# bkpcoding/distributed_ML_pytorch

Measured on AMD Instinct MI355X. Metric: samples/sec (whole node) ResNet-18 ASGD at 1/2/4/8 MI355X; time-to-target-loss, higher is better.
Workload: dtype bf16; 1 GPU; model=resnet18 (CIFAR stem), global_batch=512, per_gpu_batch=512, image=3x32x32, parallelism=asgd-local-ps x1, n_push=10, n_pull=10, staleness=1, push_combine=sum, hip_graph=True, master_dtype=fp32, wire_dtype=fp32

## Files before the change

### distributed_ml_pytorch_amd/csrc/bind/conv.cpp

```cpp
#include "util.h"

namespace dmp::bind {
namespace {

struct ConvGeom {
  int B, CI, H, W, CO, R, S, OH, OW;
};

ConvGeom geom_of(const Tensor& x, const Tensor& w, int64_t OH, int64_t OW) {
  return {(int)x.size(0), (int)x.size(1), (int)x.size(2), (int)x.size(3), (int)w.size(0),
          (int)w.size(2), (int)w.size(3), (int)OH, (int)OW};
}

bool halo_takes(int64_t cfg, int H, int W, int C, int R, int S, int64_t stride, int64_t pad) {
  return cfg >= dmp::conv_halo_base() && cfg < dmp::conv_halo_base() + dmp::conv_num_halo_configs() &&
         stride == 1 && pad == 1 &&
         dmp::conv_halo_ok((int)cfg, H, W, C, R, S, (int)stride, (int)pad);
}

ConvGeom conv_geom(const Tensor& x, const Tensor& w, int64_t stride, int64_t pad,
                   int64_t halo_cfg = -1) {
  TORCH_CHECK(x.dim() == 4 && w.dim() == 4, "conv: 4-D tensors expected");
  TORCH_CHECK(w.size(1) == x.size(1), "conv: weight/input channel mismatch");
  TORCH_CHECK(stride >= 1 && pad >= 0, "conv: bad stride/pad");
// ... 360 lines not shown
  return config_table(dmp::conv_num_configs(), dmp::conv_config_info, 5);
}

std::vector<int64_t> conv_halo_configs(int64_t H, int64_t W, int64_t C, int64_t R, int64_t S,
                                       int64_t stride, int64_t pad) {
  std::vector<int64_t> out;
  config_ids(out, dmp::conv_halo_base(), dmp::conv_num_halo_configs(), [&](int c) {
    return dmp::conv_halo_ok(c, (int)H, (int)W, (int)C, (int)R, (int)S, (int)stride, (int)pad);
  });
  return out;
}

std::vector<int64_t> conv_dgrad_s2_configs(int64_t H, int64_t W, int64_t OH, int64_t OW,
                                           int64_t CO, int64_t CI, int64_t R, int64_t S,
                                           int64_t stride, int64_t pad) {
  std::vector<int64_t> out;
  config_ids(out, dmp::conv_dgrad_s2_base(), dmp::conv_dgrad_s2_num_configs(), [&](int c) {
    return dmp::conv_dgrad_s2_ok(c, (int)H, (int)W, (int)OH, (int)OW, (int)CO, (int)CI, (int)R,
                                 (int)S, (int)stride, (int)pad);
  });
  return out;
}

std::vector<int64_t> conv_wgrad_halo_configs(int64_t B, int64_t H, int64_t W, int64_t CI,
                                             int64_t CO, int64_t R, int64_t S, int64_t stride,
                                             int64_t pad) {
  std::vector<int64_t> out;
  for (int base : {dmp::conv_wgrad_halo_base(), dmp::conv_wgrad_halo_slab_base()})
    config_ids(out, base, dmp::conv_wgrad_num_halo_configs(), [&](int c) {
      return dmp::conv_wgrad_halo_ok(c, (int)B, (int)H, (int)W, (int)CI, (int)CO, (int)R, (int)S,
                                     (int)stride, (int)pad);
    });
  return out;
}

}

void bind_conv(pybind11::module_& m) {
  m.def("conv_fwd", &conv_fwd, "NHWC bf16 implicit-GEMM conv forward (+BN partials)",
        py::arg("x"), py::arg("w"), py::arg("stride"), py::arg("pad"), py::arg("want_stats"),
        py::arg("cfg") = -1, py::arg("slots") = py::none(), py::arg("bias") = py::none(),
        py::arg("relu") = false, py::arg("addend") = py::none());
  m.def("conv_dgrad", &conv_dgrad, "NHWC bf16 implicit-GEMM conv data gradient", py::arg("dy"),
        py::arg("w"), py::arg("H"), py::arg("W"), py::arg("stride"), py::arg("pad"),
        py::arg("cfg") = -1, py::arg("wt") = py::none(), py::arg("addend") = py::none(),
        py::arg("addend_sub") = false, py::arg("addend_mask") = py::none());
  m.def("subsample2", &subsample2, "x[:, :, ::2, ::2] of a channels_last bf16 activation",
        py::arg("x"));
  m.def("add_subsampled2", &add_subsampled2, "dx[:, :, ::2, ::2] += xs in place",
        py::arg("dx"), py::arg("xs"));
  m.def("conv_weight_transpose_batched", &conv_weight_transpose_batched,
        "transpose every conv weight of a flat bf16 shadow in one launch");
  m.def("conv_wgrad", &conv_wgrad, "NHWC bf16 conv weight gradient (fp32 accumulate)",
        py::arg("dy"), py::arg("x"), py::arg("dw"), py::arg("stride"), py::arg("pad"),
        py::arg("cfg") = -1, py::arg("dbias") = py::none());
  m.def("conv_configs", &conv_configs, "[(id, BM, BN, BK, threads)] of the compiled conv tiles");
  m.def("conv_wgrad_halo_configs", &conv_wgrad_halo_configs,
        "3x3 stride-1 / stride-2 halo wgrad cfg ids applicable to (B, H, W, CI, CO, R, S, stride, pad)");
  m.def("conv_dgrad_s2_configs", &conv_dgrad_s2_configs,
        "3x3/stride-2 halo data-gradient cfg ids for (H, W, OH, OW, CO, CI, R, S, stride, pad)");
  m.def("conv_halo_configs", &conv_halo_configs,
        "3x3/stride-1 halo-tile cfg ids applicable to (H, W, C, R, S, stride, pad)");
  m.def("conv_halo_pm", [](bool on) { return dmp::conv_halo_pm(on); },
        "position-major halo tiles on 4 x 4 maps: set the process-wide switch, return the "
        "previous value (never inside a graph capture)", py::arg("on"));
  m.def("conv_halo_pm_ok",
        [](int64_t cfg, int64_t H, int64_t W, int64_t C, int64_t R, int64_t S, int64_t stride,
           int64_t pad) {
          return dmp::conv_halo_pm_ok((int)cfg, (int)H, (int)W, (int)C, (int)R, (int)S, (int)stride,
                                      (int)pad);
        },
        "halo cfg id runs position-major on (H, W, C, R, S, stride, pad) when the switch is on");
  m.def("stem_supported", [](int64_t H, int64_t W) { return dmp::stem_supported((int)H, (int)W); },
        "ImageNet 7x7/2 stem kernel applies to an H x W input");
  m.def("stem_fwd", &stem_fwd, "ImageNet stem conv forward (+BN partials) via space-to-depth",
        py::arg("x"), py::arg("w"), py::arg("want_stats"), py::arg("slots") = py::none(),
        py::arg("bias") = py::none(), py::arg("relu") = false);
  m.def("stem_wgrad", &stem_wgrad, "ImageNet stem conv weight gradient (fp32 +=)", py::arg("dy"),
        py::arg("xs"), py::arg("dw"));
  m.def("conv_small_fwd", &conv_small_fwd, "few-input-channel conv forward (+BN partials)",
        py::arg("x"), py::arg("w"), py::arg("stride"), py::arg("pad"), py::arg("want_stats"),
        py::arg("slots") = py::none());
  m.def("conv_small_wgrad", &conv_small_wgrad, "few-input-channel conv weight gradient (fp32 +=)",
        py::arg("dy"), py::arg("x"), py::arg("dw"), py::arg("stride"), py::arg("pad"));
  m.def("stem3_route", &stem3_route,
        "conv_small_fwd / conv_small_wgrad run the MFMA stem kernels for this geometry",
        py::arg("CI"), py::arg("R"), py::arg("S"), py::arg("CO"), py::arg("stride"),
        py::arg("pad"), py::arg("W"));
  m.def("stem3_bn_bwd_scratch_floats", [] { return (int64_t)dmp::stem3_bn_bwd_scratch_floats(); },
        "fp32 elements of stem3_bn_bwd's persistent scratch");
  m.def("stem3_bn_bwd", &stem3_bn_bwd,
        "CIFAR stem: BN + ReLU backward and conv weight gradient in one pass (all +=)",
        py::arg("dy"), py::arg("x0"), py::arg("x"), py::arg("stats"), py::arg("gamma"),
        py::arg("dgamma"), py::arg("dbeta"), py::arg("dw"), py::arg("scratch"),
        py::arg("zero_buf") = py::none(), py::arg("blocks") = 0);
  m.def("im2col", &im2col, "NHWC patch rows [B*OH*OW, Kp], k = (r, s, ci), zero-padded",
        py::arg("x"), py::arg("R"), py::arg("S"), py::arg("stride"), py::arg("pad"), py::arg("Kp"));
  m.def("col2im", &col2im, "gather-form inverse of im2col -> channels_last dX", py::arg("dcols"),
        py::arg("B"), py::arg("CI"), py::arg("H"), py::arg("W"), py::arg("R"), py::arg("S"),
        py::arg("stride"), py::arg("pad"));
}

}
```

### distributed_ml_pytorch_amd/csrc/conv_wgrad.hip

```cpp
#include "common.h"
#include "halo_plan.h"
#include "mfma_prims.h"

#ifndef DMP_ABLATE
#define DMP_ABLATE 0
#endif

namespace dmp {


struct WgradArgs {
  const u16* dy;
  const u16* x;
  float* dw;
  int B, GH, GW, CI, OH, OW, CO, R, S, stride, pad;
  long long P;
  int p_chunk;
  float* dbias;
  float* slab;
  int xcd;
};

template <int ROWE>
__device__ __forceinline__ int wg_f(int row) {
  if constexpr (ROWE == 128) return (row & 3) | (((row >> 3) & 1) << 2);
  else return ((row >> 1) & 1) | (((row >> 3) & 1) << 1);
}
template <int ROWE>
__device__ __forceinline__ int wg_off(int row, int col) {
  return row * ROWE + ((((col >> 4) ^ wg_f<ROWE>(row))) << 4) + (col & 15);
}

// ... 398 lines not shown
    float* park = reinterpret_cast<float*>(lds_w);
    if (grp == 1) {
#pragma unroll
      for (int t = 0; t < NT; ++t)
#pragma unroll
        for (int i = 0; i < 4; ++i)
          *reinterpret_cast<f32x4*>(park + ((wc * NT * 4 + t * 4 + i) * 64 + lane) * 4) = acc[t][i];
    }
    __syncthreads();
    if (grp == 1) return;
#pragma unroll
    for (int t = 0; t < NT; ++t)
#pragma unroll
      for (int i = 0; i < 4; ++i)
        acc[t][i] += *reinterpret_cast<const f32x4*>(park + ((wc * NT * 4 + t * 4 + i) * 64 + lane) * 4);
  }
  const long long K = 9LL * C;
  const int ci = ci0 + wc * 16 + (lane & 15);
#pragma unroll
  for (int t = 0; t < NT; ++t)
#pragma unroll
    for (int i = 0; i < 4; ++i)
#pragma unroll
      for (int rr = 0; rr < 4; ++rr) {
        const int co = co0 + i * 16 + 4 * (lane >> 4) + rr;
        float* dst = a.dw + (long long)co * K + ((r0 + t / 3) * 3 + t % 3) * C + ci;
        if (atomic == 1) atomicAdd(dst, acc[t][i][rr]);
        else if (atomic == 0) *dst += acc[t][i][rr];
        else if (atomic == 3) a.slab[(long long)bz * CO * K + (dst - a.dw)] = acc[t][i][rr];
        else *dst = acc[t][i][rr];
      }
}

bool conv_wgrad_halo_ok(int cfg, int B, int H, int W, int CI, int CO, int R, int S, int stride,
                        int pad) {
  const WgradHaloPlan p = plan_wgrad_halo(cfg, B, H, W, CI, CO, R, S, stride, pad);
  return p.ok && (cfg < kWhSlabBase || p.slab_elems > 0);
}
long long conv_wgrad_halo_slab_elems(int cfg, int B, int H, int W, int CI, int CO, int R, int S,
                                     int stride, int pad) {
  return plan_wgrad_halo(cfg, B, H, W, CI, CO, R, S, stride, pad).slab_elems;
}
int conv_wgrad_halo_base() { return kWhBase; }
int conv_wgrad_halo_slab_base() { return kWhSlabBase; }
int conv_wgrad_num_halo_configs() { return kNumWhConfigs; }

__global__ void __launch_bounds__(256) wgrad_slab_reduce_kernel(const float* __restrict__ slab,
                                                                float* __restrict__ dw,
                                                                long long n4, int splits) {
  __shared__ float4 red[16][16];
  const int lx = threadIdx.x & 15, ly = threadIdx.x >> 4;
  const long long v = (long long)blockIdx.x * 16 + lx;
  const float4* s4 = reinterpret_cast<const float4*>(slab);
  float4 t = {0.f, 0.f, 0.f, 0.f};
  if (v < n4) {
    int sp = ly;
#pragma unroll 4
    for (; sp < splits; sp += 16) {
      const float4 u = s4[sp * n4 + v];
      t.x += u.x; t.y += u.y; t.z += u.z; t.w += u.w;
    }
  }
  red[ly][lx] = t;
  __syncthreads();
  if (ly == 0 && v < n4) {
#pragma unroll
// ... 11 lines not shown
static void launch_wgrad_halo_t(const WgradArgs& a, const WgradHaloGeom& g, size_t lds, int splits,
                                hipStream_t s) {
  static int diag = -1;
  allow_max_dynamic_lds<conv_wgrad_halo_kernel<BM, NS, TR, PG, S2>>();
  if (diag < 0) {
    const char* e = getenv("DMP_WGRAD_HALO_DIAG");
    diag = (e && e[0] == 's') ? 1 : 0;
  }
  const dim3 grid((unsigned)(a.CI / 64), (unsigned)(a.CO / 64 * (3 / TR)), (unsigned)splits);
  const int mode = diag ? 2 : (splits > 1 ? (a.slab != nullptr ? 3 : 1) : 0);
  hipLaunchKernelGGL((conv_wgrad_halo_kernel<BM, NS, TR, PG, S2>), grid, dim3(256 * PG), lds, s, a,
                     g, mode);
  if (mode == 3) {
    const long long n4 = (long long)a.CO * 9 * a.CI / 4;
    hipLaunchKernelGGL(wgrad_slab_reduce_kernel, dim3((unsigned)((n4 + 15) / 16)), dim3(256), 0,
                       s, a.slab, a.dw, n4, splits);
  }
}

template <int NS, int TR>
static void launch_wgrad_halo_bm(int bm, const WgradArgs& a, const WgradHaloGeom& g, size_t lds,
                                 int sp, hipStream_t s) {
  if constexpr (TR == 1) {
    if (bm == 224) {
      launch_wgrad_halo_t<224, NS, 1>(a, g, lds, sp, s);
      return;
    }
  }
  if (bm == 64) launch_wgrad_halo_t<64, NS, TR>(a, g, lds, sp, s);
  else if (TR == 3 || bm == 128) launch_wgrad_halo_t<128, NS, TR>(a, g, lds, sp, s);
  else launch_wgrad_halo_t<(TR == 3 ? 128 : 256), NS, TR>(a, g, lds, sp, s);
}

template <int BNW, int WM, int WN, int BMW = 64>
static void launch_wgrad_variant(const WgradArgs& a, dim3 grid, int bp, int ns, hipStream_t s) {
  if (bp == 32) {
    if (ns == 3) hipLaunchKernelGGL((conv_wgrad_kernel<BNW, WM, WN, 32, 3, BMW>), grid, dim3(256), 0, s, a);
    else hipLaunchKernelGGL((conv_wgrad_kernel<BNW, WM, WN, 32, 2, BMW>), grid, dim3(256), 0, s, a);
  } else {
    if (ns == 3) hipLaunchKernelGGL((conv_wgrad_kernel<BNW, WM, WN, 64, 3, BMW>), grid, dim3(256), 0, s, a);
    else hipLaunchKernelGGL((conv_wgrad_kernel<BNW, WM, WN, 64, 2, BMW>), grid, dim3(256), 0, s, a);
  }
}

void launch_conv_wgrad(const u16* dy, const u16* x, float* dw, int B, int H, int W, int CI,
                       int OH, int OW, int CO, int R, int S, int stride, int pad, int cfg,
                       hipStream_t s, float* dbias, float* slab) {
  WgradArgs a{dy, x, dw, B, H, W, CI, OH, OW, CO, R, S, stride, pad, (long long)B * OH * OW, 0,
              dbias, nullptr};
  if (cfg >= kWhSlabBase) {
    if (slab != nullptr) a.slab = slab;
    else cfg -= kWhSlabBase - kWhBase;
  }
  if (cfg >= kWhBase && dbias == nullptr) {
    if (const WgradHaloPlan p = plan_wgrad_halo(cfg, B, H, W, CI, CO, R, S, stride, pad); p.ok) {
      const WgradHaloGeom& g = p.g;
      const int bm = p.bm, ns = p.ns, tr = p.tr, pg = p.pg, sp = p.splits;
      const size_t lds = p.lds;
      if (stride == 2) {
        if (pg == 2) {
          if (bm == 128) launch_wgrad_halo_t<128, 2, 1, 2, true>(a, g, lds, sp, s);
          else launch_wgrad_halo_t<256, 2, 1, 2, true>(a, g, lds, sp, s);
        } else if (ns == 2) {
          if (bm == 64) launch_wgrad_halo_t<64, 2, 1, 1, true>(a, g, lds, sp, s);
          else if (bm == 128) launch_wgrad_halo_t<128, 2, 1, 1, true>(a, g, lds, sp, s);
          else launch_wgrad_halo_t<256, 2, 1, 1, true>(a, g, lds, sp, s);
        } else {
          if (bm == 64) launch_wgrad_halo_t<64, 3, 1, 1, true>(a, g, lds, sp, s);
          else if (bm == 128) launch_wgrad_halo_t<128, 3, 1, 1, true>(a, g, lds, sp, s);
          else launch_wgrad_halo_t<256, 3, 1, 1, true>(a, g, lds, sp, s);
        }
        return;
      }
      if (pg == 2) {
        if (bm == 128) launch_wgrad_halo_t<128, 2, 1, 2>(a, g, lds, sp, s);
        else launch_wgrad_halo_t<256, 2, 1, 2>(a, g, lds, sp, s);
      } else if (tr == 3) {
        if (ns == 2) launch_wgrad_halo_bm<2, 3>(bm, a, g, lds, sp, s);
        else launch_wgrad_halo_bm<3, 3>(bm, a, g, lds, sp, s);
      } else {
        if (ns == 2) launch_wgrad_halo_bm<2, 1>(bm, a, g, lds, sp, s);
        else if (ns == 3) launch_wgrad_halo_bm<3, 1>(bm, a, g, lds, sp, s);
        else launch_wgrad_halo_bm<4, 1>(bm, a, g, lds, sp, s);
      }
      return;
// ... 36 lines not shown
```

### distributed_ml_pytorch_amd/csrc/halo_plan.h

```cpp
#pragma once

#include <cstddef>

#include "halo_pm.h"

namespace dmp {

constexpr int kMaxDynamicLds = 160 * 1024;

struct HaloGeom {
  int TH, TB, HROWS, A_INS, MV;
  int W2, PI, PSW;
};

struct HaloPGeom {
  int TH, TB, HROWS, APW, AINS, ntiles;
  int xform;
  float xs, xh, xlo;
  int stagger;
};

struct WgradHaloGeom {
  int TH, TB, THX, XROWS, XPW, ntiles, tiles_per_split, MV;
};

constexpr int kHaloAPW = 8;
constexpr int kHpAPW = 12;
constexpr int hp_apw_max(int nw) { return nw == 8 ? 8 : kHpAPW; }
constexpr int kWhXPW = 12;

struct HaloTiling {
  bool ok;
  int TH, TB, MV;
};

inline HaloTiling halo_tiling(int bm, int H, int W, bool padded) {
  HaloTiling t{};
// ... 239 lines not shown
  if (stride != 1 && !(s2 && tr == 1 && H % 2 == 0 && W % 2 == 0 && ns <= 3 && kWhBM[var] == 0))
    return p;
  if (tr == 3 && bm > 128) return p;
  const int XW = W;
  if (s2) { H /= 2; W /= 2; }
  const HaloTiling t = halo_tiling(bm, H, W, true);
  if (!t.ok) return p;
  WgradHaloGeom& h = p.g;
  h.TH = t.TH;
  h.TB = t.TB;
  h.MV = t.MV;
  h.THX = h.TH + tr - 1;
  h.XROWS = h.TB * h.THX * (XW + 2);
  h.XPW = ((h.XROWS + 7) / 8 + 4 * pg - 1) / (4 * pg);
  if (h.XPW > kWhXPW || h.THX + 1 > 127 || h.TB > 0x7fff) return p;
  if ((ns - 2) * (bm / 32 + h.XPW) > 40) return p;
  const long long M = (long long)B * H * W;
  if (2LL * M * (CO > CI ? CO : CI) * (s2 ? 4 : 1) >= (1LL << 31)) return p;
  h.ntiles = (int)((M + h.MV - 1) / h.MV);
  const int per = (CI / 64) * (CO / 64) * (3 / tr);
  int sp = target / per;
  if (sp < 1) sp = 1;
  if (sp > h.ntiles) sp = h.ntiles;
  h.tiles_per_split = (h.ntiles + sp - 1) / sp;
  p.splits = (h.ntiles + h.tiles_per_split - 1) / h.tiles_per_split;
  const size_t stage = (size_t)bm * 64 + (size_t)h.XPW * 4 * pg * 512;
  p.lds = (size_t)ns * stage * 2;
  p.ok = p.lds <= (size_t)kMaxDynamicLds;
  if (p.ok && slab && p.splits > 1 && wh_slab_variant(var))
    p.slab_elems = (long long)p.splits * CO * R * S * CI;
  return p;
}

}
```

### distributed_ml_pytorch_amd/csrc/launchers.h

```cpp
#pragma once
#include <hip/hip_runtime_api.h>

#include "bn_slots.h"
#include <stdint.h>

namespace dmp {

void launch_asgd_fused_step(const float* g, float* p, float* acc, float* mom, uint16_t* w16,
                            long long n, float lr, float wd, float momentum, float dampening,
                            bool nesterov, hipStream_t s);
int optim_hyper_words();
void launch_optim_hyper(float* hyper, const float* g, float* partial, long long n, hipStream_t s);
void launch_asgd_fused_step_dev(const float* g, float* p, float* acc, float* mom, uint16_t* w16,
                                long long n, const float* hyper, float wd, float momentum,
                                float dampening, bool nesterov, hipStream_t s);
void launch_adamw_fused_step(const float* g, float* p, float* acc, float* m, float* v,
                             uint16_t* w16, const uint8_t* decay, long long n, const float* hyper,
                             float wd, float eps, hipStream_t s);
struct Wire {
  enum Kind { kF32, kBF16, kMX8 } kind;
  const void* data;
};
void launch_ps_apply(float* shard, Wire delta, uint16_t* mirror, long long n, float scale,
                     bool atomic, hipStream_t s, const float* factor = nullptr);
// ... 136 lines not shown
void launch_dropout_mask(uint8_t* mask, long long nmask, float p, unsigned long long seed,
                         const long long* offset, hipStream_t s);
void launch_dropout_apply_bf16(const uint16_t* x, const uint8_t* mask, uint16_t* y, long long n,
                               float scale, int mode, long long inner, int C, hipStream_t s);
void launch_dropout_apply_f32(const float* x, const uint8_t* mask, float* y, long long n,
                              float scale, int mode, long long inner, int C, hipStream_t s);

void launch_drop_path_draw(float* table, long long* state, const long long* thr,
                           const float* scale, int branches, int B, unsigned long long seed,
                           hipStream_t s);
void launch_drop_path_rows(const uint16_t* x, const float* rscale, uint16_t* y, long long per,
                           long long nvec, hipStream_t s);

int conv_num_configs();
void conv_config_info(int cfg, int* info);
int conv_default_config(long long M, int CO);
int conv_fwd_num_mblocks(long long M, int CO, int cfg);
int conv_num_halo_configs();
bool conv_dgrad_s2_ok(int cfg, int H, int W, int OH, int OW, int K, int N, int R, int S, int stride,
                      int pad);
int conv_dgrad_s2_base();
int conv_dgrad_s2_num_configs();
int conv_halo_base();
bool conv_halo_ok(int cfg, int H, int W, int C, int R, int S, int stride, int pad);
bool conv_halo_pm(bool on);
bool conv_halo_pm_ok(int cfg, int H, int W, int C, int R, int S, int stride, int pad);
int conv_wgrad_halo_base();
int conv_wgrad_num_halo_configs();
bool conv_wgrad_halo_ok(int cfg, int B, int H, int W, int CI, int CO, int R, int S, int stride,
                        int pad);
int conv_wgrad_halo_slab_base();
long long conv_wgrad_halo_slab_elems(int cfg, int B, int H, int W, int CI, int CO, int R, int S,
                                     int stride, int pad);
void launch_conv_fwd(const uint16_t* x, const uint16_t* w, uint16_t* y, float* part, int B, int H,
                     int W, int CI, int OH, int OW, int CO, int R, int S, int stride, int pad,
                     int cfg, hipStream_t s, const float* bias = nullptr, bool relu = false,
                     const uint16_t* addend = nullptr);
void launch_conv_dgrad(const uint16_t* dy, const uint16_t* wt, uint16_t* dx, int B, int H, int W,
                       int CI, int OH, int OW, int CO, int R, int S, int stride, int pad, int cfg,
                       hipStream_t s, const uint16_t* addend = nullptr, bool addend_sub = false,
                       const uint8_t* addend_mask = nullptr);
void launch_subsample2(const uint16_t* x, uint16_t* xs, int B, int H, int W, int C,
                       hipStream_t s);
void launch_add_subsampled2(uint16_t* dx, const uint16_t* xs, int B, int H, int W, int C,
                            hipStream_t s);
void launch_conv_weight_transpose(const uint16_t* w, uint16_t* wt, int CO, int RS, int CI,
                                  hipStream_t s);
void launch_conv_wgrad(const uint16_t* dy, const uint16_t* x, float* dw, int B, int H, int W,
                       int CI, int OH, int OW, int CO, int R, int S, int stride, int pad, int cfg,
                       hipStream_t s, float* dbias = nullptr, float* slab = nullptr);

bool stem3_supported(int CI, int R, int S, int CO, int stride, int pad, int W);
void launch_stem3_fwd(const uint16_t* x, int xbytes, int sb, int sh, int sw, int sc,
                      const uint16_t* w, uint16_t* y, float* part, int B, int H, int W, int CI,
                      hipStream_t s);
void launch_stem3_wgrad(const uint16_t* dy, const uint16_t* x, int xbytes, int sb, int sh, int sw,
                        int sc, float* dw, int B, int H, int W, int CI, hipStream_t s);
int stem3_bn_bwd_scratch_floats();
int stem3_bn_bwd_steps(long long P, int target);
long long stem3_bn_bwd_blocks(long long P, int target);
void launch_stem3_bn_bwd(const uint16_t* dy, const uint16_t* x0, const uint16_t* x, int xbytes,
                         int sb, int sh, int sw, int sc, const float* stats, const float* gamma,
                         float* dgamma, float* dbeta, float* dw, float* scratch, float* zero_buf,
                         int B, int H, int W, int CI, int blocks, hipStream_t s);
int conv_small_max_k();
long long conv_small_fwd_blocks(long long P);
// ... 61 lines not shown
```

Before: 146,700 samples/s.

## Add position-major halo weight-gradient kernel for 4x4 and 8x8 maps

Adds a new 3x3 stride-1 wgrad kernel for 4x4 and 8x8 feature maps. It stages tiles position-major, grouping 32 images per column, and skips MFMAs for dead padding taps, so only (3W-2)^2 of the 9W^2 products are computed. Work is split across row offsets with its own split planner and slab reduction. Reads go through transposed LDS reads with an XOR swizzle meant to avoid bank conflicts. It is on by default through an env switch and routes eligible halo configs away from the existing halo kernel, at the cost of more code paths and a new planner that could pick poorer splits.

```diff
diff --git a/distributed_ml_pytorch_amd/csrc/bind/conv.cpp b/distributed_ml_pytorch_amd/csrc/bind/conv.cpp
--- a/distributed_ml_pytorch_amd/csrc/bind/conv.cpp
+++ b/distributed_ml_pytorch_amd/csrc/bind/conv.cpp
@@ -416,6 +416,15 @@
                                      (int)stride, (int)pad);
     });
   return out;
+}
+
+bool conv_wgrad_pm_ok(int64_t cfg, int64_t B, int64_t H, int64_t W, int64_t CI, int64_t CO,
+                      int64_t R, int64_t S, int64_t stride, int64_t pad) {
+  if (std::max({cfg, B, H, W, CI, CO, R, S, stride, pad}) >= (int64_t(1) << 30) ||
+      std::min({cfg, B, H, W, CI, CO, R, S, stride, pad}) < 0)
+    return false;
+  return dmp::conv_wgrad_pm_ok((int)cfg, (int)B, (int)H, (int)W, (int)CI, (int)CO, (int)R, (int)S,
+                               (int)stride, (int)pad);
 }
 
 }
@@ -455,6 +464,13 @@
                                       (int)pad);
         },
         "halo cfg id runs position-major on (H, W, C, R, S, stride, pad) when the switch is on");
+  m.def("conv_wgrad_pm", [](bool on) { return dmp::conv_wgrad_pm(on); },
+        "position-major halo weight gradient on 4 x 4 / 8 x 8 maps: set the process-wide "
+        "switch, return the previous value (never inside a graph capture)", py::arg("on"));
+  m.def("conv_wgrad_pm_ok", &conv_wgrad_pm_ok,
+        "halo wgrad cfg id runs position-major on (B, H, W, CI, CO, R, S, stride, pad) when the "
+        "switch is on", py::arg("cfg"), py::arg("B"), py::arg("H"), py::arg("W"), py::arg("CI"),
+        py::arg("CO"), py::arg("R"), py::arg("S"), py::arg("stride"), py::arg("pad"));
   m.def("stem_supported", [](int64_t H, int64_t W) { return dmp::stem_supported((int)H, (int)W); },
         "ImageNet 7x7/2 stem kernel applies to an H x W input");
   m.def("stem_fwd", &stem_fwd, "ImageNet stem conv forward (+BN partials) via space-to-depth",
diff --git a/distributed_ml_pytorch_amd/csrc/conv_wgrad.hip b/distributed_ml_pytorch_amd/csrc/conv_wgrad.hip
--- a/distributed_ml_pytorch_amd/csrc/conv_wgrad.hip
+++ b/distributed_ml_pytorch_amd/csrc/conv_wgrad.hip
@@ -1,3 +1,6 @@
+#include <cstdlib>
+#include <type_traits>
+
 #include "common.h"
 #include "halo_plan.h"
 #include "mfma_prims.h"
@@ -462,6 +465,207 @@
       }
 }
 
+template <int A, int B, class F>
+__device__ __forceinline__ void static_for(F&& f) {
+  if constexpr (A < B) {
+    f(std::integral_constant<int, A>{});
+    static_for<A + 1, B>(f);
+  }
+}
+
+template <int W, int PG>
+__global__ void __launch_bounds__(256 * PG) conv_wgrad_halo_pm_kernel(WgradArgs a, WgradPmGeom pg,
+                                                                      int atomic) {
+  constexpr int H = W, NW = 4 * PG, CW = 64, BM = wpm::tile_rows(W);
+  constexpr int PW = wpm::dma_pieces(W) / NW;
+  constexpr int D_EL = BM * CW, STAGE = 2 * D_EL;
+  static_assert(wpm::map_ok(W) && wpm::dma_pieces(W) % NW == 0, "whole DMA pieces per wave");
+  extern __shared__ __attribute__((aligned(16))) u16 lds_w[];
+
+  const int tid = threadIdx.x, lane = tid & 63;
+  const int wid = __builtin_amdgcn_readfirstlane(tid >> 6);
+  const int wc = wid & 3, grp = wid >> 2;
+  const int nx = gridDim.x, ny = gridDim.y, G = nx * ny * gridDim.z;
+  const int bid = blockIdx.x + nx * (blockIdx.y + ny * blockIdx.z);
+  const int xcd = bid & 7, q8 = G >> 3, r8 = G & 7;
+  const int lid = (xcd < r8 ? xcd * (q8 + 1) : r8 * (q8 + 1) + (xcd - r8) * q8) + (bid >> 3);
+  const int bx = lid % nx, by = (lid / nx) % ny, bz = lid / (nx * ny);
+  const int ci0 = bx * CW, co0 = by * CW;
+  int r0 = 0, ks = bz, sp = pg.sp[0];
+  if (ks >= sp) {
+    ks -= sp; r0 = 1; sp = pg.sp[1];
+    if (ks >= sp) { ks -= sp; r0 = 2; sp = pg.sp[2]; }
+  }
+  const int nh = wpm::n_h(H, r0), hlo = wpm::h_lo(r0), ntl = pg.G * nh;
+  const int t_begin = wpm::run_begin(ks, sp, ntl), t_end = wpm::run_begin(ks + 1, sp, ntl);
+  const int C = a.CI, CO = a.CO;
+
+  unsigned d_rel[PW], x_rel[PW];
+#pragma unroll
+  for (int j = 0; j < PW; ++j) {
+    const int row = (wid + j * NW) * 8 + lane / 8, pch = lane % 8;
+    const int pix = wpm::row_img(row) * H * W + wpm::row_col(row), ch = wpm::dma_chan(row, pch);
+    d_rel[j] = 2u * (unsigned)(pix * CO + co0 + ch);
+    x_rel[j] = 2u * (unsigned)(pix * C + ci0 + ch);
+  }
+  const __amdgpu_buffer_rsrc_t rsD = __builtin_amdgcn_make_buffer_rsrc(
+      (void*)a.dy, 0, (int)(2LL * a.B * H * W * CO), 0x00020000);
+  const __amdgpu_buffer_rsrc_t rsX = __builtin_amdgcn_make_buffer_rsrc(
+      (void*)a.x, 0, (int)(2LL * a.B * H * W * C), 0x00020000);
+
+  int cg = t_begin / nh, chh = hlo + (t_begin - cg * nh);
+  auto stage = [&](int buf, int t) {
+    u16* Ds = lds_w + buf * STAGE;
+    u16* Xs = Ds + D_EL;
+    const bool live = t < t_end;
+    const int pb = (cg * wpm::kGroup * H + chh) * W;
+    if (++chh == hlo + nh) { chh = hlo; ++cg; }
+    const unsigned dbase = 2u * (unsigned)(pb * CO);
+    const unsigned xbase = 2u * (unsigned)((pb + (r0 - 1) * W) * C);
+#pragma unroll
+    for (int j = 0; j < PW; ++j)
+      dma16(rsD, live ? d_rel[j] + dbase : kOOB, Ds + (wid + j * NW) * 512);
+#pragma unroll
+    for (int j = 0; j < PW; ++j)
+      dma16(rsX, live ? x_rel[j] + xbase : kOOB, Xs + (wid + j * NW) * 512);
+  };
+
+  const int li = lane & 15, pc = li & 3;
+  int a_off[2][4], x_off[2];
+#pragma unroll
+  for (int hs = 0; hs < 2; ++hs) {
+    const int k = wpm::lane_k(lane, hs);
+#pragma unroll
+    for (int i = 0; i < 4; ++i) a_off[hs][i] = wpm::lds_off(k, i * 16 + 4 * pc);
+    x_off[hs] = wpm::lds_off(k, wc * 16 + 4 * pc);
+  }
+  auto tr = [&](const u16* p) -> s16x4_t {
+    return __builtin_amdgcn_ds_read_tr16_b64_v4i16((__attribute__((address_space(3))) s16x4_t*)p);
+  };
+
+  f32x4 acc[3][4];
+#pragma unroll
+  for (int s = 0; s < 3; ++s)
+#pragma unroll
+    for (int i = 0; i < 4; ++i) acc[s][i] = f32x4{0.f, 0.f, 0.f, 0.f};
+
+  auto compute = [&](int buf, auto w0c, auto w1c) {
+    constexpr int W0 = decltype(w0c)::value, W1 = decltype(w1c)::value;
+    const u16* Ds = lds_w + buf * STAGE;
+    const u16* Xs = Ds + D_EL;
+    bf16x8 af[2][4], xf[W];
+    auto load_a = [&](int w, int slot) {
+#pragma unroll
+      for (int i = 0; i < 4; ++i) {
+        const s16x4_t lo = tr(Ds + w * wpm::kGroup * CW + a_off[0][i]);
+        const s16x4_t hi = tr(Ds + w * wpm::kGroup * CW + a_off[1][i]);
+        af[slot][i] = __builtin_bit_cast(bf16x8, __builtin_shufflevector(lo, hi, 0, 1, 2, 3, 4, 5, 6, 7));
+      }
+    };
+    auto load_x = [&](int c) {
+      const s16x4_t lo = tr(Xs + c * wpm::kGroup * CW + x_off[0]);
+      const s16x4_t hi = tr(Xs + c * wpm::kGroup * CW + x_off[1]);
+      xf[c] = __builtin_bit_cast(bf16x8, __builtin_shufflevector(lo, hi, 0, 1, 2, 3, 4, 5, 6, 7));
+    };
+    constexpr int C0 = W0 > 0 ? W0 - 1 : 0, C1 = W0 + 1 < W ? W0 + 1 : W - 1;
+    load_a(W0, 0);
+    static_for<C0, C1 + 1>([&](auto c) { load_x(decltype(c)::value); });
+    __builtin_amdgcn_sched_group_barrier(0x100, 8 + 2 * (C1 - C0 + 1), 0);
+    static_for<W0, W1>([&](auto wv) {
+      constexpr int w = decltype(wv)::value, slot = (w - W0) & 1;
+      constexpr bool more = w + 1 < W1, morex = more && w + 2 < W;
+      constexpr int NRD = more ? 8 + (morex ? 2 : 0) : 0, NMF = 4 * wpm::live_taps(W, w);
+      if constexpr (more) load_a(w + 1, slot ^ 1);
+      if constexpr (morex) load_x(w + 2);
+      static_for<0, 3>([&](auto sv) {
+        constexpr int s = decltype(sv)::value;
+        if constexpr (wpm::tap_live(W, w, s)) {
+#pragma unroll
+          for (int i = 0; i < 4; ++i) acc[s][i] = mfma16(af[slot][i], xf[w + s - 1], acc[s][i]);
+        }
+      });
+      static_for<0, NMF>([&](auto m) {
+        __builtin_amdgcn_sched_group_barrier(0x008, 1, 0);
+        if constexpr (decltype(m)::value < NRD) __builtin_amdgcn_sched_group_barrier(0x100, 1, 0);
+      });
+      if constexpr (NRD > NMF) __builtin_amdgcn_sched_group_barrier(0x100, NRD - NMF, 0);
+    });
+  };
+
+  using std::integral_constant;
+  const int nt = t_end - t_begin;
+  if (nt > 0) stage(0, t_begin);
+  for (int it = 0; it < nt; ++it) {
+    wait_vm<0>();
+    __builtin_amdgcn_s_barrier();
+    asm volatile("" ::: "memory");
+    stage((it + 1) & 1, t_begin + it + 1);
+    if constexpr (PG == 1) {
+      compute(it & 1, integral_constant<int, 0>{}, integral_constant<int, W>{});
+    } else {
+      if (grp == 0) compute(it & 1, integral_constant<int, 0>{}, integral_constant<int, W / 2>{});
+      else compute(it & 1, integral_constant<int, W / 2>{}, integral_constant<int, W>{});
+    }
+  }
+  wait_vm<0>();
+  if constexpr (PG == 2) {
+    __syncthreads();
+    float* park = reinterpret_cast<float*>(lds_w);
+    if (grp == 1) {
+#pragma unroll
+      for (int t = 0; t < 3; ++t)
+#pragma unroll
+        for (int i = 0; i < 4; ++i)
+          *reinterpret_cast<f32x4*>(park + ((wc * 12 + t * 4 + i) * 64 + lane) * 4) = acc[t][i];
+    }
+    __syncthreads();
+    if (grp == 1) return;
+#pragma unroll
+    for (int t = 0; t < 3; ++t)
+#pragma unroll
+      for (int i = 0; i < 4; ++i)
+        acc[t][i] += *reinterpret_cast<const f32x4*>(park + ((wc * 12 + t * 4 + i) * 64 + lane) * 4);
+  }
+  const long long K = 9LL * C;
+  const int ci = ci0 + wc * 16 + (lane & 15);
+#pragma unroll
+  for (int t = 0; t < 3; ++t)
+#pragma unroll
+    for (int i = 0; i < 4; ++i)
+#pragma unroll
+      for (int rr = 0; rr < 4; ++rr) {
+        const int co = co0 + i * 16 + 4 * (lane >> 4) + rr;
+        const long long e = (long long)co * K + (r0 * 3 + t) * C + ci;
+        if (atomic == 1) atomicAdd(a.dw + e, acc[t][i][rr]);
+        else if (atomic == 0) a.dw[e] += acc[t][i][rr];
+        else {
+          a.slab[(long long)ks * CO * K + e] = acc[t][i][rr];
+          if (ks == sp - 1)
+            for (int z = sp; z < pg.spmax; ++z) a.slab[(long long)z * CO * K + e] = 0.f;
+        }
+      }
+}
+
+static bool& wgrad_pm_switch() {
+  static bool on = [] {
+    const char* e = std::getenv("DMP_WGRAD_PM");
+    return e == nullptr || e[0] != '0';
+  }();
+  return on;
+}
+
+bool conv_wgrad_pm(bool on) {
+  bool& sw = wgrad_pm_switch();
+  const bool prev = sw;
+  sw = on;
+  return prev;
+}
+
+bool conv_wgrad_pm_ok(int cfg, int B, int H, int W, int CI, int CO, int R, int S, int stride,
+                      int pad) {
+  return plan_wgrad_halo_pm(cfg, B, H, W, CI, CO, R, S, stride, pad).ok;
+}
+
 bool conv_wgrad_halo_ok(int cfg, int B, int H, int W, int CI, int CO, int R, int S, int stride,
                         int pad) {
   const WgradHaloPlan p = plan_wgrad_halo(cfg, B, H, W, CI, CO, R, S, stride, pad);
@@ -539,6 +743,21 @@
   else launch_wgrad_halo_t<(TR == 3 ? 128 : 256), NS, TR>(a, g, lds, sp, s);
 }
 
+template <int W, int PG>
+static void launch_wgrad_pm_t(WgradArgs a, const WgradPmPlan& p, hipStream_t s) {
+  allow_max_dynamic_lds<conv_wgrad_halo_pm_kernel<W, PG>>();
+  const WgradPmGeom& g = p.g;
+  if (p.slab_elems == 0) a.slab = nullptr;
+  const dim3 grid((unsigned)(a.CI / 64), (unsigned)(a.CO / 64), (unsigned)(2 * g.sp[0] + g.sp[1]));
+  const int mode = a.slab != nullptr ? 3 : (g.spmax > 1 ? 1 : 0);
+  hipLaunchKernelGGL((conv_wgrad_halo_pm_kernel<W, PG>), grid, dim3(256 * PG), p.lds, s, a, g, mode);
+  if (mode == 3) {
+    const long long n4 = (long long)a.CO * 9 * a.CI / 4;
+    hipLaunchKernelGGL(wgrad_slab_reduce_kernel, dim3((unsigned)((n4 + 15) / 16)), dim3(256), 0,
+                       s, a.slab, a.dw, n4, g.spmax);
+  }
+}
+
 template <int BNW, int WM, int WN, int BMW = 64>
 static void launch_wgrad_variant(const WgradArgs& a, dim3 grid, int bp, int ns, hipStream_t s) {
   if (bp == 32) {
@@ -558,6 +777,18 @@
   if (cfg >= kWhSlabBase) {
     if (slab != nullptr) a.slab = slab;
     else cfg -= kWhSlabBase - kWhBase;
+  }
+  if (cfg >= kWhBase && dbias == nullptr && wgrad_pm_switch()) {
+    if (const WgradPmPlan p = plan_wgrad_halo_pm(cfg, B, H, W, CI, CO, R, S, stride, pad); p.ok) {
+      if (W == 4) {
+        if (p.pg == 2) launch_wgrad_pm_t<4, 2>(a, p, s);
+        else launch_wgrad_pm_t<4, 1>(a, p, s);
+      } else {
+        if (p.pg == 2) launch_wgrad_pm_t<8, 2>(a, p, s);
+        else launch_wgrad_pm_t<8, 1>(a, p, s);
+      }
+      return;
+    }
   }
   if (cfg >= kWhBase && dbias == nullptr) {
     if (const WgradHaloPlan p = plan_wgrad_halo(cfg, B, H, W, CI, CO, R, S, stride, pad); p.ok) {
diff --git a/distributed_ml_pytorch_amd/csrc/halo_plan.h b/distributed_ml_pytorch_amd/csrc/halo_plan.h
--- a/distributed_ml_pytorch_amd/csrc/halo_plan.h
+++ b/distributed_ml_pytorch_amd/csrc/halo_plan.h
@@ -3,6 +3,7 @@
 #include <cstddef>
 
 #include "halo_pm.h"
+#include "wgrad_pm.h"
 
 namespace dmp {
 
@@ -308,4 +309,55 @@
   return p;
 }
 
-}
+struct WgradPmGeom {
+  int G;
+  int sp[3];
+  int spmax;
+};
+
+struct WgradPmPlan {
+  bool ok;
+  WgradPmGeom g;
+  int W, pg, q;
+  int blocks;
+  size_t lds;
+  long long slab_elems;
+};
+
+constexpr bool wgrad_pm_variant(int var) { return var == 0 || var == 5; }
+
+inline WgradPmPlan plan_wgrad_halo_pm(int cfg, int B, int H, int W, int CI, int CO, int R, int S,
+                                      int stride, int pad) {
+  WgradPmPlan p{};
+  const bool slab = cfg >= kWhSlabBase;
+  const int id = cfg - (slab ? kWhSlabBase : kWhBase);
+  if (id < 0 || id >= kNumWhConfigs || !wgrad_pm_variant(id / 12)) return p;
+  if (R != 3 || S != 3 || stride != 1 || pad != 1 || H != W || !wpm::map_ok(W)) return p;
+  const WgradHaloPlan d = plan_wgrad_halo(cfg, B, H, W, CI, CO, R, S, stride, pad);
+  if (!d.ok || d.bm != wpm::tile_rows(W) || d.ns != 2 || d.tr != 1) return p;
+  p.W = W;
+  p.pg = d.pg;
+  WgradPmGeom& g = p.g;
+  g.G = (B + wpm::kGroup - 1) / wpm::kGroup;
+  if (2LL * g.G * wpm::kGroup * H * W * (CO > CI ? CO : CI) >= (1LL << 31)) return p;
+  const int n0 = wpm::live_tiles(g.G, H, 0), n1 = wpm::live_tiles(g.G, H, 1);
+  const int cap = 3 * d.splits;
+  for (int q = (2 * n0 + n1 + cap - 1) / cap; q <= n1 && !p.ok; ++q) {
+    const int s0 = (n0 + q - 1) / q, s1 = (n1 + q - 1) / q;
+    if ((long long)s0 * (q - 1) > n0 || (long long)s1 * (q - 1) > n1 || 2 * s0 + s1 > cap) continue;
+    g.sp[0] = g.sp[2] = s0;
+    g.sp[1] = s1;
+    g.spmax = s1 > s0 ? s1 : s0;
+    p.q = q;
+    p.ok = true;
+  }
+  if (!p.ok) return p;
+  p.blocks = (CI / 64) * (CO / 64) * (2 * g.sp[0] + g.sp[1]);
+  p.lds = (size_t)2 * 2 * wpm::tile_rows(W) * 64 * 2;
+  p.ok = p.lds <= (size_t)kMaxDynamicLds;
+  if (p.ok && slab && d.slab_elems > 0 && g.spmax > 1 && g.spmax <= d.splits)
+    p.slab_elems = (long long)g.spmax * CO * R * S * CI;
+  return p;
+}
+
+}
diff --git a/distributed_ml_pytorch_amd/csrc/launchers.h b/distributed_ml_pytorch_amd/csrc/launchers.h
--- a/distributed_ml_pytorch_amd/csrc/launchers.h
+++ b/distributed_ml_pytorch_amd/csrc/launchers.h
@@ -192,6 +192,9 @@
 int conv_wgrad_halo_slab_base();
 long long conv_wgrad_halo_slab_elems(int cfg, int B, int H, int W, int CI, int CO, int R, int S,
                                      int stride, int pad);
+bool conv_wgrad_pm(bool on);
+bool conv_wgrad_pm_ok(int cfg, int B, int H, int W, int CI, int CO, int R, int S, int stride,
+                      int pad);
 void launch_conv_fwd(const uint16_t* x, const uint16_t* w, uint16_t* y, float* part, int B, int H,
                      int W, int CI, int OH, int OW, int CO, int R, int S, int stride, int pad,
                      int cfg, hipStream_t s, const float* bias = nullptr, bool relu = false,
diff --git a/distributed_ml_pytorch_amd/csrc/wgrad_pm.h b/distributed_ml_pytorch_amd/csrc/wgrad_pm.h
--- /dev/null
+++ b/distributed_ml_pytorch_amd/csrc/wgrad_pm.h
@@ -0,0 +1,44 @@
+#pragma once
+
+namespace dmp {
+namespace wpm {
+
+constexpr int kGroup = 32;
+constexpr bool map_ok(int W) { return W == 4 || W == 8; }
+constexpr int tile_rows(int W) { return kGroup * W; }
+
+constexpr int h_lo(int r) { return r == 0 ? 1 : 0; }
+constexpr int n_h(int H, int r) { return r == 1 ? H : H - 1; }
+constexpr int live_tiles(int G, int H, int r) { return G * n_h(H, r); }
+constexpr int run_begin(int k, int sp, int n) { return (int)(((long long)k * n) / sp); }
+
+constexpr bool tap_live(int W, int w, int s) { return w + s - 1 >= 0 && w + s - 1 < W; }
+constexpr int live_taps(int W, int w) {
+  return (tap_live(W, w, 0) ? 1 : 0) + 1 + (tap_live(W, w, 2) ? 1 : 0);
+}
+constexpr int live_products(int W) {
+  int n = 0;
+  for (int r = 0; r < 3; ++r)
+    for (int w = 0; w < W; ++w) n += n_h(W, r) * live_taps(W, w);
+  return n;
+}
+static_assert(live_products(4) == 100 && live_products(8) == 484, "(3W - 2)^2");
+
+constexpr int staged_row(int i, int w) { return w * kGroup + i; }
+constexpr int row_img(int row) { return row % kGroup; }
+constexpr int row_col(int row) { return row / kGroup; }
+constexpr int dma_pieces(int W) { return tile_rows(W) / 8; }
+constexpr int swz(int row) { return ((row >> 1) & 1) | (((row >> 3) & 1) << 1); }
+constexpr int lds_off(int row, int col) {
+  return row * 64 + (((col >> 4) ^ swz(row)) << 4) + (col & 15);
+}
+constexpr int dma_chan(int row, int pch) { return (((pch >> 1) ^ swz(row)) << 4) + (pch & 1) * 8; }
+
+constexpr int lane_k(int lane, int hsel) { return 8 * (lane >> 4) + ((lane & 15) >> 2) + 4 * hsel; }
+constexpr int lane_c(int lane) { return 4 * (lane & 3); }
+
+constexpr int step_lo(int W, int pg, int grp) { return grp * W / pg; }
+constexpr int step_hi(int W, int pg, int grp) { return (grp + 1) * W / pg; }
+
+}
+}
diff --git a/distributed_ml_pytorch_amd/csrc/wgrad_pm_check.cpp b/distributed_ml_pytorch_amd/csrc/wgrad_pm_check.cpp
--- /dev/null
+++ b/distributed_ml_pytorch_amd/csrc/wgrad_pm_check.cpp
@@ -0,0 +1,311 @@
+#include <cstdio>
+#include <cstdlib>
+#include <vector>
+
+#include "halo_plan.h"
+
+using namespace dmp;
+
+static long long g_checks = 0;
+static int g_failed = 0;
+
+#define CHECK(cond, ...)                               \
+  do {                                                 \
+    ++g_checks;                                        \
+    if (!(cond)) {                                     \
+      ++g_failed;                                      \
+      std::printf("FAIL %s:%d: ", __FILE__, __LINE__); \
+      std::printf(__VA_ARGS__);                        \
+      std::printf("\n");                               \
+    }                                                  \
+  } while (0)
+
+constexpr unsigned kOOB = 0x80000000u;
+
+static int pm_cfg(int W, int pg, int spl, bool slab) {
+  const int var = pg == 2 ? 5 : 0, bm_sel = W == 4 ? 1 : 2;
+  return (slab ? kWhSlabBase : kWhBase) + var * 12 + bm_sel * 4 + spl;
+}
+
+static int check_liveness(int W) {
+  const int H = W;
+  std::vector<int> hit((size_t)H * W * 9, 0);
+  for (int r = 0; r < 3; ++r)
+    for (int j = 0; j < wpm::live_tiles(1, H, r); ++j) {
+      const int h = wpm::h_lo(r) + j % wpm::n_h(H, r);
+      CHECK(j / wpm::n_h(H, r) == 0 && h >= 0 && h < H, "tile %d of tap row %d", j, r);
+      for (int w = 0; w < W; ++w)
+        for (int s = 0; s < 3; ++s)
+          if (wpm::tap_live(W, w, s)) ++hit[((size_t)h * W + w) * 9 + r * 3 + s];
+    }
+  int live = 0;
+  for (int h = 0; h < H; ++h)
+    for (int w = 0; w < W; ++w)
+      for (int t = 0; t < 9; ++t) {
+        const int hh = h + t / 3 - 1, ww = w + t % 3 - 1;
+        const bool ref = hh >= 0 && hh < H && ww >= 0 && ww < W;
+        CHECK(hit[((size_t)h * W + w) * 9 + t] == (ref ? 1 : 0), "W %d pixel (%d, %d) tap %d: %d", W,
+              h, w, t, hit[((size_t)h * W + w) * 9 + t]);
+        live += ref ? 1 : 0;
+      }
+  CHECK(live == wpm::live_products(W) && live == (3 * W - 2) * (3 * W - 2), "live products %d", live);
+  std::printf("W %d: %d of %d (pixel, tap) products live\n", W, live, 9 * H * W);
+  return live;
+}
+
+static bool block_run(const WgradPmGeom& g, int H, int bz, int* r0, int* ks, int* tb, int* te) {
+  int r = 0, k = bz, sp = g.sp[0];
+  if (k >= sp) {
+    k -= sp; r = 1; sp = g.sp[1];
+    if (k >= sp) { k -= sp; r = 2; sp = g.sp[2]; }
+  }
+  if (k >= sp) return false;
+  const int n = wpm::live_tiles(g.G, H, r);
+  *r0 = r;
+  *ks = k;
+  *tb = wpm::run_begin(k, sp, n);
+  *te = wpm::run_begin(k + 1, sp, n);
+  return true;
+}
+
+static void check_runs(int cfg, int B, int W, int CI, int CO, bool print) {
+  const int H = W;
+  const WgradPmPlan p = plan_wgrad_halo_pm(cfg, B, H, W, CI, CO, 3, 3, 1, 1);
+  const WgradHaloPlan d = plan_wgrad_halo(cfg, B, H, W, CI, CO, 3, 3, 1, 1);
+  if (print)
+    std::printf("plan cfg %d B %d W %d %dx%d: %s sp %d/%d/%d q %d blocks %d (dense %d) flush %lld KB "
+                "(dense %lld KB)\n", cfg, B, W, CI, CO, p.ok ? "pm" : "dense", p.g.sp[0], p.g.sp[1],
+                p.g.sp[2], p.q, p.blocks, d.ok ? (CI / 64) * (CO / 64) * 3 * d.splits : 0,
+                48LL * p.blocks, d.ok ? 48LL * (CI / 64) * (CO / 64) * 3 * d.splits : 0);
+  if (!p.ok) return;
+  const WgradPmGeom& g = p.g;
+  CHECK(d.ok && p.blocks <= (CI / 64) * (CO / 64) * 3 * d.splits, "cfg %d: %d blocks, dense %d", cfg,
+        p.blocks, d.ok ? (CI / 64) * (CO / 64) * 3 * d.splits : -1);
+  CHECK(g.G == (B + 31) / 32 && g.spmax >= g.sp[0] && g.spmax >= g.sp[1] && g.spmax >= g.sp[2],
+        "geometry");
+  CHECK(p.lds == (size_t)2 * 2 * wpm::tile_rows(W) * 64 * 2 && p.lds <= (size_t)kMaxDynamicLds &&
+            (p.pg == 1 || p.lds >= (size_t)4 * 12 * 64 * 16), "LDS %zu", p.lds);
+  if (p.slab_elems > 0)
+    CHECK(p.slab_elems <= d.slab_elems && p.slab_elems == (long long)g.spmax * CO * 9 * CI,
+          "slab %lld of %lld", p.slab_elems, d.slab_elems);
+  std::vector<int> seen((size_t)3 * g.G * H, 0);
+  int lo = 1 << 30, hi = 0, nb = 0, r0, ks, tb, te;
+  for (int bz = 0; block_run(g, H, bz, &r0, &ks, &tb, &te); ++bz) {
+    ++nb;
+    const int cnt = te - tb;
+    if (cnt < lo) lo = cnt;
+    if (cnt > hi) hi = cnt;
+    for (int t = tb; t < te; ++t) {
+      const int gi = t / wpm::n_h(H, r0), h = wpm::h_lo(r0) + t % wpm::n_h(H, r0);
+      CHECK(gi < g.G && h + r0 - 1 >= 0 && h + r0 - 1 < H, "tile (%d, %d, %d)", r0, gi, h);
+      if (gi < g.G && h < H) ++seen[((size_t)r0 * g.G + gi) * H + h];
+    }
+  }
+  CHECK(nb == 2 * g.sp[0] + g.sp[1] && nb * (CI / 64) * (CO / 64) == p.blocks, "%d blocks", nb);
+  CHECK(lo >= 1 && hi - lo <= 1 && hi == p.q, "cfg %d B %d W %d: runs of %d..%d tiles (q %d)", cfg, B, W,
+        lo, hi, p.q);
+  for (int r = 0; r < 3; ++r)
+    for (int gi = 0; gi < g.G; ++gi)
+      for (int h = 0; h < H; ++h) {
+        const bool live = h + r - 1 >= 0 && h + r - 1 < H;
+        CHECK(seen[((size_t)r * g.G + gi) * H + h] == (live ? 1 : 0), "tile (%d, %d, %d) run %d times",
+              r, gi, h, seen[((size_t)r * g.G + gi) * H + h]);
+      }
+}
+
+static void tr_read(const std::vector<int>& lds, const int* addr, int out[64][4]) {
+  for (int l = 0; l < 64; ++l) {
+    const int g = l >> 4, i = l & 15;
+    for (int q = 0; q < 4; ++q) {
+      const size_t e = (size_t)addr[16 * g + 4 * q + i / 4] + i % 4;
+      if (e >= lds.size() || (e - i % 4) % 4 != 0)
+        CHECK(false, "tr read at element %zu of the stage", e - i % 4);
+      out[l][q] = e < lds.size() ? lds[e] : 0;
+    }
+  }
+}
+
+static void check_wgrad(int B, int W, int pg) {
+  const int H = W, C = 64, CO = 64, HW = H * W, NW = 4 * pg, PW = wpm::dma_pieces(W) / NW;
+  const int cfg = pm_cfg(W, pg, 0, false);
+  const WgradPmPlan plan = plan_wgrad_halo_pm(cfg, B, H, W, C, CO, 3, 3, 1, 1);
+  CHECK(plan.ok && plan.pg == pg && plan.W == W, "plan_wgrad_halo_pm refuses cfg %d at B %d", cfg, B);
+  if (!plan.ok) return;
+  const WgradPmGeom& g = plan.g;
+  const int BM = wpm::tile_rows(W), D_EL = BM * 64;
+  CHECK(wpm::dma_pieces(W) % NW == 0 && (size_t)2 * 2 * D_EL * 2 == plan.lds, "stage size");
+
+  std::vector<int> x((size_t)B * HW * C), dy((size_t)B * HW * CO);
+  unsigned sd = 2463534242u + (unsigned)(B * 64 + W * 4 + pg);
+  auto rnd = [&] { sd = sd * 1664525u + 1013904223u; return (int)((sd >> 24) % 7) - 3; };
+  for (auto& v : x) v = rnd();
+  for (auto& v : dy) v = rnd();
+  std::vector<long long> ref((size_t)CO * 9 * C, 0), dw((size_t)CO * 9 * C, 0);
+  for (int b = 0; b < B; ++b)
+    for (int h = 0; h < H; ++h)
+      for (int w = 0; w < W; ++w)
+        for (int t = 0; t < 9; ++t) {
+          const int hh = h + t / 3 - 1, ww = w + t % 3 - 1;
+          if (hh < 0 || hh >= H || ww < 0 || ww >= W) continue;
+          for (int co = 0; co < CO; ++co)
+            for (int ci = 0; ci < C; ++ci)
+              ref[((size_t)co * 9 + t) * C + ci] += dy[((size_t)b * HW + h * W + w) * CO + co] *
+                                                    x[((size_t)b * HW + hh * W + ww) * C + ci];
+        }
+  const unsigned nrD = 2u * (unsigned)(B * HW * CO), nrX = 2u * (unsigned)(B * HW * C);
+  auto fetch = [&](const std::vector<int>& src, unsigned nr, unsigned off, int e) {
+    if (off >= nr) return 0;
+    CHECK(off % 16 == 0 && off + 16 <= nr, "DMA offset %u of %u", off, nr);
+    return src[off / 2 + e];
+  };
+  long long mfmas = 0;
+  int r0, ks, tb, te;
+  for (int bz = 0; block_run(g, H, bz, &r0, &ks, &tb, &te); ++bz) {
+    const int nh = wpm::n_h(H, r0), hlo = wpm::h_lo(r0);
+    int cg = tb / nh, chh = hlo + (tb - cg * nh);
+    for (int t = tb; t < te; ++t) {
+      std::vector<int> Ds((size_t)D_EL, 777), Xs((size_t)D_EL, 777);
+      const int pb = (cg * wpm::kGroup * H + chh) * W;
+      if (++chh == hlo + nh) { chh = hlo; ++cg; }
+      const unsigned dbase = 2u * (unsigned)(pb * CO), xbase = 2u * (unsigned)((pb + (r0 - 1) * W) * C);
+      for (int wid = 0; wid < NW; ++wid)
+        for (int j = 0; j < PW; ++j)
+          for (int lane = 0; lane < 64; ++lane) {
+            const int row = (wid + j * NW) * 8 + lane / 8, pch = lane % 8;
+            CHECK(row < BM, "DMA row %d", row);
+            const int pix = wpm::row_img(row) * HW + wpm::row_col(row), ch = wpm::dma_chan(row, pch);
+            const unsigned d_rel = 2u * (unsigned)(pix * CO + ch), x_rel = 2u * (unsigned)(pix * C + ch);
+            CHECK(d_rel + dbase < kOOB && x_rel + xbase < kOOB, "offset wraps");
+            for (int e = 0; e < 8; ++e) {
+              const size_t dst = (size_t)(wid + j * NW) * 512 + lane * 8 + e;
+              Ds[dst] = fetch(dy, nrD, d_rel + dbase, e);
+              Xs[dst] = fetch(x, nrX, x_rel + xbase, e);
+            }
+          }
+      for (int wid = 0; wid < NW; ++wid) {
+        const int wc = wid & 3, grp = wid >> 2;
+        for (int w = wpm::step_lo(W, pg, grp); w < wpm::step_hi(W, pg, grp); ++w) {
+          int af[4][64][8], xf[3][64][8];
+          for (int hs = 0; hs < 2; ++hs) {
+            int addr[64], out[64][4];
+            for (int i = 0; i < 4; ++i) {
+              for (int l = 0; l < 64; ++l)
+                addr[l] = w * wpm::kGroup * 64 + wpm::lds_off(wpm::lane_k(l, hs), i * 16 + wpm::lane_c(l));
+              tr_read(Ds, addr, out);
+              for (int l = 0; l < 64; ++l)
+                for (int q = 0; q < 4; ++q) af[i][l][4 * hs + q] = out[l][q];
+            }
+            for (int s = 0; s < 3; ++s) {
+              if (!wpm::tap_live(W, w, s)) continue;
+              for (int l = 0; l < 64; ++l)
+                addr[l] = (w + s - 1) * wpm::kGroup * 64 +
+                          wpm::lds_off(wpm::lane_k(l, hs), wc * 16 + wpm::lane_c(l));
+              tr_read(Xs, addr, out);
+              for (int l = 0; l < 64; ++l)
+                for (int q = 0; q < 4; ++q) xf[s][l][4 * hs + q] = out[l][q];
+            }
+          }
+          for (int s = 0; s < 3; ++s) {
+            if (!wpm::tap_live(W, w, s)) continue;
+            for (int i = 0; i < 4; ++i) {
+              ++mfmas;
+              for (int m = 0; m < 16; ++m)
+                for (int n = 0; n < 16; ++n) {
+                  long long acc = 0;
+                  for (int gq = 0; gq < 4; ++gq)
+                    for (int k = 0; k < 8; ++k) acc += af[i][16 * gq + m][k] * xf[s][16 * gq + n][k];
+                  dw[((size_t)(i * 16 + m) * 9 + r0 * 3 + s) * C + wc * 16 + n] += acc;
+                }
+            }
+          }
+        }
+      }
+    }
+  }
+  long long bad = 0;
+  for (size_t e = 0; e < ref.size(); ++e) bad += dw[e] != ref[e];
+  CHECK(bad == 0, "wgrad B=%d W=%d PG=%d: %lld wrong elements", B, W, pg, bad);
+  CHECK(mfmas == 4LL * 4 * wpm::live_products(W) * g.G, "B=%d W=%d PG=%d: %lld MFMAs", B, W, pg, mfmas);
+}
+
+static int half_degree(const int* addr_el, int half) {
+  int banks[64] = {}, worst = 0;
+  for (int l = 32 * half; l < 32 * half + 32; ++l)
+    for (int k = 0; k < 2; ++k) {
+      const int d = ++banks[(addr_el[l] * 2 / 4 + k) % 64];
+      if (d > worst) worst = d;
+    }
+  return worst;
+}
+
+static int check_conflicts(int W, int* reads) {
+  int worst = 0, addr[64];
+  for (int w = 0; w < W; ++w)
+    for (int hs = 0; hs < 2; ++hs) {
+      for (int i = 0; i < 4; ++i) {
+        for (int l = 0; l < 64; ++l)
+          addr[l] = w * wpm::kGroup * 64 + wpm::lds_off(wpm::lane_k(l, hs), i * 16 + wpm::lane_c(l));
+        for (int half = 0; half < 2; ++half) {
+          const int d = half_degree(addr, half);
+          if (d > worst) worst = d;
+        }
+        ++*reads;
+      }
+      for (int wc = 0; wc < 4; ++wc) {
+        for (int l = 0; l < 64; ++l)
+          addr[l] = w * wpm::kGroup * 64 + wpm::lds_off(wpm::lane_k(l, hs), wc * 16 + wpm::lane_c(l));
+        for (int half = 0; half < 2; ++half) {
+          const int d = half_degree(addr, half);
+          if (d > worst) worst = d;
+        }
+        ++*reads;
+      }
+    }
+  for (int row = 0; row < wpm::tile_rows(W); ++row)
+    for (int pch = 0; pch < 8; ++pch) {
+      const int ch = wpm::dma_chan(row, pch);
+      CHECK(wpm::lds_off(row, ch) == row * 64 + pch * 8, "DMA chunk (%d, %d) vs lds_off", row, pch);
+      CHECK(wpm::swz(row) == wpm::swz(row % wpm::kGroup), "swizzle key depends on the column");
+    }
+  return worst;
+}
+
+int main() {
+  const int l4 = check_liveness(4), l8 = check_liveness(8);
+  for (int base : {kWhBase, kWhSlabBase})
+    for (int i = 0; i < kNumWhConfigs; ++i) {
+      const int var = i / 12, bm = kWhBM[var] ? kWhBM[var] : 64 << (i % 12 / 4);
+      for (int W : {4, 8, 16}) {
+        const WgradPmPlan p = plan_wgrad_halo_pm(base + i, 33, W, W, 128, 128, 3, 3, 1, 1);
+        const bool want = (var == 0 || var == 5) && bm == 32 * W && W != 16;
+        CHECK(p.ok == want, "cfg %d on %d x %d: %d", base + i, W, W, (int)p.ok);
+        if (p.ok) CHECK(plan_wgrad_halo(base + i, 33, W, W, 128, 128, 3, 3, 1, 1).ok, "no dense plan");
+      }
+      CHECK(!plan_wgrad_halo_pm(base + i, 33, 8, 8, 128, 128, 3, 3, 2, 1).ok, "stride 2 accepted");
+      CHECK(!plan_wgrad_halo_pm(base + i, 33, 4, 8, 128, 128, 3, 3, 1, 1).ok, "4 x 8 accepted");
+      CHECK(!plan_wgrad_halo_pm(base + i, 33, 4, 4, 128, 128, 1, 1, 1, 0).ok, "1 x 1 accepted");
+    }
+  CHECK(!plan_wgrad_halo_pm(pm_cfg(4, 1, 0, false), 1 << 20, 4, 4, 512, 512, 3, 3, 1, 1).ok,
+        "oversize batch accepted");
+  for (int W : {4, 8})
+    for (int pg : {1, 2})
+      for (int B : {1, 32, 33}) check_wgrad(B, W, pg);
+  for (int W : {4, 8})
+    for (int pg : {1, 2})
+      for (int spl = 0; spl < 4; ++spl)
+        for (bool slab : {false, true}) {
+          const int cfg = pm_cfg(W, pg, spl, slab);
+          for (int B : {1, 31, 32, 33, 65, 100, 1000})
+            for (int ch : {64, 128, 256}) check_runs(cfg, B, W, ch, ch, false);
+          const int ch = W == 4 ? 512 : 256;
+          check_runs(cfg, 64, W, ch, ch, !slab);
+          check_runs(cfg, 512, W, ch, ch, !slab);
+        }
+  int reads4 = 0, reads8 = 0;
+  const int deg4 = check_conflicts(4, &reads4), deg8 = check_conflicts(8, &reads8);
+  std::printf("tr reads per tile: %d (4 x 4), %d (8 x 8)\n", reads4, reads8);
+  CHECK(deg4 == 1 && deg8 == 1, "bank conflicts");
+  std::printf("wgrad_pm_check: %lld checks, %d failed, live %d/144 %d/576, tr-read conflict degree %d %d\n",
+              g_checks, g_failed, l4, l8, deg4, deg8);
+  return g_failed ? 1 : 0;
+}
```

After: 147,100 samples/s, median of 3. No clear change (+0.3%).
